# Wu-sm/Adversarial-Attacks-on-GAN-based-Image-Fusion

Hardware: AMD Instinct MI355X
Metric: attacked images/sec, PGD-20 L∞ ε=8/255 at 256², 1/2/4/8 MI355X (higher is better)
Workload: dtype f32; 1 GPU; PGD-20 L∞ eps=8/255 alpha=2/255 at 256², 128 images/GPU (BASELINE config #4 per-GPU share), RCCL all-gather of outputs when N>1; encoder=e4e, norm=linf, images_per_gpu=128, global_batch=128, size=256, pgd_steps=20, parallelism=dp1, dist_world_size=1, output_in_eps_ball_and_finite=True, fp32_arithmetic=fp32

## Files before the change

adversarial-attacks-on-gan-based-image-fusion_amd/csrc/conv_halo_x6.hip:

```cpp
#include "conv_common.h"
#include "halo_epilogue.h"

namespace mia {

#ifdef MIA_STAMPS
__device__ unsigned long long g_x6_stamps[4][16];
#endif

template <int BN_, int TPS_ = 1>
struct HaloX6 {
  static constexpr int PH = 16, PW = 16, NW = 8, NT = 64 * NW;
  static constexpr int WN = BN_ == 128 ? 2 : 1, WM = NW / WN, FM = 16 / WM, FN = 4;
  static constexpr int BM = PH * PW, BN = BN_, BK = 32;
  static constexpr int HSIDE = PW + 2, HROWS = (PH + 2) * HSIDE;
  static constexpr int HPIECES = (HROWS + 7) / 8;
  static constexpr int HBUF = HPIECES * 1024;
  static constexpr int LROWB = 64, LBUF = HROWS * LROWB;
  static constexpr int TPS = TPS_, NG = (9 + TPS - 1) / TPS;
  static constexpr int BHM = BN * ROWB, BL = BN * LROWB, BSTAGE1 = BHM + BL;
  static constexpr int BSTAGE = TPS * BSTAGE1;
  static constexpr int BWAVES = 4, HWAVES = 4;
  static constexpr int B_HM_INS = BN / 8 / BWAVES;
  static constexpr int B_L_INS = BN / 16 / BWAVES;
  static constexpr int H_INS = (HPIECES + HWAVES - 1) / HWAVES;
  static constexpr int HSTEPS = (4 + TPS - 1) / TPS;
  static constexpr int H_PER_STEP = (H_INS + HSTEPS - 1) / HSTEPS;
  static constexpr int EROWS = 128, ES = BN + 4;
  static constexpr int LDS = 2 * HBUF + LBUF + 2 * BSTAGE;
  static_assert(WM * FM * 16 == BM && WN * FN * 16 == BN, "");
  static_assert(B_HM_INS * 8 * BWAVES == BN && B_L_INS * 16 * BWAVES == BN, "");
  static_assert(LDS <= 160 * 1024, "");
};

template <int BN_, bool PRO, int EPI, bool EARLY, bool PRIO, bool UNR, int TPS = 1>
__global__ __launch_bounds__(HaloX6<BN_>::NT, 2) void conv_halo_x6_kernel(const ConvK k) {
  static_assert(!UNR || (EARLY && PRIO && EPI != -2), "UNR: the EARLY + PRIO schedule, D[ch][px]");
  static_assert(UNR || TPS == 1, "several taps per K-step: the unrolled loop only");
  typedef HaloX6<BN_, TPS> TL;
  constexpr int NG = TL::NG;
  constexpr int FM = TL::FM, FN = TL::FN, WN = TL::WN, NT = TL::NT, BN = TL::BN, BK = TL::BK;
  constexpr int HSIDE = TL::HSIDE, HROWS = TL::HROWS, HPIECES = TL::HPIECES, HBUF = TL::HBUF;
  constexpr int H_INS = TL::H_INS, HPS = TL::H_PER_STEP, HWAVES = TL::HWAVES;
  constexpr int B_HM_INS = TL::B_HM_INS, B_L_INS = TL::B_L_INS, BSTAGE = TL::BSTAGE;

  extern __shared__ __attribute__((aligned(16))) char smem[];
  char* const hbuf = smem;
  char* const lbuf = smem + 2 * HBUF;
  char* const bring = lbuf + TL::LBUF;

  const mia_conv_args& p = k.a;
  const int tid = threadIdx.x, lane = tid & 63;
  const int wid = __builtin_amdgcn_readfirstlane(tid >> 6);
  const int wm = wid / WN, wn = wid % WN;
  const ConvGroup G = k.g[0];
  const int H = p.H, W = p.W, Cin = p.Cin, Cout = p.Cout, Kpad = G.kpad;
  const int bl = xcd_remap(blockIdx.x, k.nblk);
  const int mt = bl / k.nbn, n0 = (bl % k.nbn) * BN;
  const int ptx = W / TL::PW, pty = H / TL::PH;
  const int x0 = (mt % ptx) * TL::PW;
  const int y0 = ((mt / ptx) % pty) * TL::PH;
  const int n = mt / (ptx * pty);

  const float* __restrict__ X = (const float*)p.x;
  const unsigned* __restrict__ Whm = (const unsigned*)G.w_split;
  const __bf16* __restrict__ Wl = (const __bf16*)(Whm + (size_t)Cout * Kpad);
  const char* zero = (const char*)g_zero16;
  const bool bwave = wid < TL::BWAVES;
  const int hw = wid - TL::BWAVES;
  const int my_pieces = bwave ? 0 : (HPIECES - hw + HWAVES - 1) / HWAVES;
#ifdef MIA_STAMPS
  const unsigned long long st_t0 = __builtin_amdgcn_s_memtime();
  const unsigned long long st_r0 = __builtin_amdgcn_s_memrealtime();
  unsigned long long st_pro = 0, st_cv = 0, st_wb = 0;
#endif

  constexpr int NSRC = H_INS > B_HM_INS + B_L_INS ? H_INS : B_HM_INS + B_L_INS;
  const char* src[NSRC];
#pragma unroll
  for (int j = 0; j < NSRC; ++j) {
    src[j] = nullptr;
    if (bwave) {
      if (j < B_HM_INS) {
        const int row = (wid * B_HM_INS + j) * 8 + (lane >> 3);
        const int c = EPI >= 0 ? min(n0 + row, Cout - 1) : n0 + row;
        if (c < Cout)
          src[j] = (const char*)(Whm + (size_t)c * Kpad + ((lane & 7) ^ fsw(row)) * 4);
      } else if (j < B_HM_INS + B_L_INS) {
        const int row = (wid * B_L_INS + j - B_HM_INS) * 16 + (lane >> 2);
        const int c = EPI >= 0 ? min(n0 + row, Cout - 1) : n0 + row;
        if (c < Cout)
          src[j] = (const char*)(Wl + (size_t)c * Kpad + ((lane & 3) ^ (lsw(row) >> 1)) * 8);
      }
    } else if (j < H_INS) {
      const int hr = (hw + HWAVES * j) * 8 + (lane >> 3);
      const int hy = hr / HSIDE, hx = hr - (hr / HSIDE) * HSIDE;
      const int y = y0 + hy - 1, x = x0 + hx - 1;
      if (hr < HROWS && y >= 0 && y < H && x >= 0 && x < W)
        src[j] = (const char*)(X + ((size_t)(n * H + y) * W + x) * Cin + ((lane & 7) ^ fsw(hr)) * 4);
    }
  }
  const int ncb = Cin / BK, nk = NG * ncb;

  auto issue_b = [&](int s, int st) {
    const int cb = s / NG, tg = s - (s / NG) * NG;
#pragma unroll
    for (int tt = 0; tt < TPS; ++tt) {
      const int t = tg * TPS + tt;
      if (TPS > 1 && t >= 9) break;
      const int koff = t * Cin + cb * BK;
      char* dst = bring + st * BSTAGE + tt * TL::BSTAGE1;
#pragma unroll
      for (int j = 0; j < B_HM_INS; ++j) {
        const char* a = EPI >= 0 ? src[j] + (size_t)koff * 4
                                 : src[j] ? src[j] + (size_t)koff * 4 : zero;
        __builtin_amdgcn_global_load_lds((gptr_t)a, (lptr_t)(dst + (wid * B_HM_INS + j) * 1024),
                                         16, 0, 0);
      }
#pragma unroll
      for (int j = 0; j < B_L_INS; ++j) {
        const char* a = EPI >= 0                ? src[B_HM_INS + j] + (size_t)koff * 2
                        : src[B_HM_INS + j] ? src[B_HM_INS + j] + (size_t)koff * 2
                                            : zero;
        __builtin_amdgcn_global_load_lds((gptr_t)a,
                                         (lptr_t)(dst + TL::BHM + (wid * B_L_INS + j) * 1024), 16,
                                         0, 0);
      }
    }
  };
  auto issue_h = [&](int cb, int j, int buf) {
    const char* a = src[j] ? src[j] + (size_t)cb * BK * 4 : zero;
    __builtin_amdgcn_global_load_lds((gptr_t)a,
                                     (lptr_t)(hbuf + buf * HBUF + (hw + HWAVES * j) * 1024), 16,
                                     0, 0);
  };
  const bool lrelu_in = p.act_in == MIA_ACT_LRELU_S2;
  auto convert = [&](int cb, int buf) {
    char* hb = hbuf + buf * HBUF;
    for (int c = tid; c < HROWS * 8; c += NT) {
      const int hr = c >> 3, pc = c & 7, lc = pc ^ fsw(hr);
      f32x4 v = *(const f32x4*)(hb + hr * ROWB + pc * 16);
      if constexpr (PRO) {
        const float mul = lrelu_in ? SQRT2 : 1.f;
        f32x4 s4 = {1.f, 1.f, 1.f, 1.f};
        if (p.in_scale) s4 = *(const f32x4*)(p.in_scale + (size_t)n * Cin + cb * BK + lc * 4);
#pragma unroll
        for (int e = 0; e < 4; ++e) {
          float f = v[e];
          if (lrelu_in) f = fmaxf(f, 0.2f * f);
          v[e] = f * (s4[e] * mul);
        }
      }
      u32x4 hm;
      u32x2 lo;
      split_quad(v, hm, lo);
      *(u32x4*)(hb + hr * ROWB + pc * 16) = hm;
      *(u32x2*)(lbuf + hr * TL::LROWB + ((lc ^ lsw(hr)) << 3)) = lo;
    }
  };

  if (bwave) {
    issue_b(0, 0);
  } else {
#pragma unroll
    for (int j = 0; j < H_INS; ++j)
      if (j < my_pieces) issue_h(0, j, 0);
  }
  asm volatile("s_waitcnt vmcnt(0)" ::: "memory");
  __syncthreads();
  convert(0, 0);
  __syncthreads();
#ifdef MIA_STAMPS
  st_pro = __builtin_amdgcn_s_memtime();
#endif

  f32x4 acc[FM][FN];
#pragma unroll
  for (int i = 0; i < FM; ++i)
#pragma unroll
    for (int j = 0; j < FN; ++j) acc[i][j] = f32x4{0.f, 0.f, 0.f, 0.f};

  const int frow = lane & 15, fq = lane >> 4;
  if constexpr (UNR) {
    int oh[FM + 2][3], ol[FM + 2][3];
#pragma unroll
    for (int q = 0; q < FM + 2; ++q)
#pragma unroll
      for (int c = 0; c < 3; ++c) {
        const int hr = (wm * FM + q) * HSIDE + frow + c;
        int vh = hr * ROWB + ((fq ^ fsw(hr)) << 4), vl = hr * TL::LROWB + ((fq ^ lsw(hr)) << 3);
        asm volatile("" : "+v"(vh), "+v"(vl));
        oh[q][c] = vh;
        ol[q][c] = vl;
      }
    int st = 0;
    for (int cb = 0; cb < ncb; ++cb) {
#pragma unroll
      for (int tg = 0; tg < NG; ++tg) {
        const int s = cb * NG + tg;
        int hoff = (cb & 1) * HBUF, x1 = 64, x2 = 32;
        asm volatile("" : "+s"(hoff), "+s"(x1), "+s"(x2));
        const char* ha = hbuf + hoff;
        const char* sb0 = bring + st * BSTAGE;
        if (bwave && s + 1 < nk) issue_b(s + 1, st ^ 1);
        if (!bwave && cb + 1 < ncb && tg < (H_INS + HPS - 1) / HPS) {
#pragma unroll
          for (int q = 0; q < HPS; ++q) {
            const int j = tg * HPS + q;
            if (j < H_INS && j < my_pieces) issue_h(cb + 1, j, (cb + 1) & 1);
          }
        }
#pragma unroll
        for (int tt = 0; tt < TPS; ++tt) {
          const int t = tg * TPS + tt;
          if (t >= 9) break;
          const int dy = t / 3, dx = t % 3;
          const char* sb = sb0 + tt * TL::BSTAGE1;
#pragma unroll
          for (int h = 0; h < 2; ++h) {
            const int ch = h * 4 + fq;
            u32x4 ahm[FM], bhm[FN];
            u32x2 al[FM], blo[FN];
#pragma unroll
            for (int i = 0; i < FM; ++i) {
              ahm[i] = *(const u32x4*)(ha + (h ? oh[i + dy][dx] ^ x1 : oh[i + dy][dx]));
              al[i] = *(const u32x2*)(lbuf + (h ? ol[i + dy][dx] ^ x2 : ol[i + dy][dx]));
            }
#pragma unroll
            for (int j = 0; j < FN; ++j) {
              const int row = wn * FN * 16 + 16 * j + frow;
              bhm[j] = *(const u32x4*)(sb + row * ROWB + ((ch ^ fsw(row)) << 4));
              blo[j] = *(const u32x2*)(sb + TL::BHM + row * TL::LROWB + ((ch ^ lsw(row)) << 3));
            }
            __builtin_amdgcn_s_setprio(1);
#pragma unroll
            for (int i = 0; i < FM; ++i)
#pragma unroll
              for (int j = 0; j < FN; ++j)
                acc[i][j] = mfma_x6(bhm[j], blo[j], ahm[i], al[i], acc[i][j]);
            __builtin_amdgcn_s_setprio(0);
          }
        }
#ifdef MIA_STAMPS
        const unsigned long long w0 = __builtin_amdgcn_s_memtime();
#endif
        if (bwave || tg == NG - 1) asm volatile("s_waitcnt vmcnt(0)" ::: "memory");
        __builtin_amdgcn_s_waitcnt(0xc07f);
        __builtin_amdgcn_s_barrier();
        __builtin_amdgcn_sched_barrier(0);
#ifdef MIA_STAMPS
        st_wb += __builtin_amdgcn_s_memtime() - w0;
#endif
        if (tg == NG - 1 && cb + 1 < ncb) {
#ifdef MIA_STAMPS
          const unsigned long long c0 = __builtin_amdgcn_s_memtime();
#endif
          convert(cb + 1, (cb + 1) & 1);
          __syncthreads();
#ifdef MIA_STAMPS
          st_cv += __builtin_amdgcn_s_memtime() - c0;
#endif
        }
        st ^= 1;
      }
    }
  } else {
  int st = 0, cb = 0, t = 0;
  for (int s = 0; s < nk; ++s) {
    const char* ha = hbuf + (cb & 1) * HBUF;
    const char* sb = bring + st * BSTAGE;
    const int dy = t >= 6 ? 2 : (t >= 3 ? 1 : 0), dx = t - 3 * dy;
    if (bwave && s + 1 < nk) issue_b(s + 1, st ^ 1);
    if constexpr (EARLY) {
      if (!bwave && cb + 1 < ncb) {
#pragma unroll
        for (int tt = 0; tt < (H_INS + HPS - 1) / HPS; ++tt) {
          if (t == tt) {
#pragma unroll
            for (int q = 0; q < HPS; ++q) {
              const int j = tt * HPS + q;
              if (j < H_INS && j < my_pieces) issue_h(cb + 1, j, (cb + 1) & 1);
            }
          }
        }
      }
    }
#pragma unroll
    for (int h = 0; h < 2; ++h) {
      const int ch = h * 4 + fq;
      u32x4 ahm[FM], bhm[FN];
      u32x2 al[FM], blo[FN];
#pragma unroll
      for (int i = 0; i < FM; ++i) {
        const int hr = (wm * FM + i + dy) * HSIDE + frow + dx;
        ahm[i] = *(const u32x4*)(ha + hr * ROWB + ((ch ^ fsw(hr)) << 4));
        al[i] = *(const u32x2*)(lbuf + hr * TL::LROWB + ((ch ^ lsw(hr)) << 3));
      }
#pragma unroll
      for (int j = 0; j < FN; ++j) {
        const int row = wn * FN * 16 + 16 * j + frow;
        bhm[j] = *(const u32x4*)(sb + row * ROWB + ((ch ^ fsw(row)) << 4));
        blo[j] = *(const u32x2*)(sb + TL::BHM + row * TL::LROWB + ((ch ^ lsw(row)) << 3));
      }
      if constexpr (PRIO) __builtin_amdgcn_s_setprio(1);
#pragma unroll
      for (int i = 0; i < FM; ++i)
#pragma unroll
        for (int j = 0; j < FN; ++j)
          acc[i][j] = EPI != -2 ? mfma_x6(bhm[j], blo[j], ahm[i], al[i], acc[i][j])
                                : mfma_x6(ahm[i], al[i], bhm[j], blo[j], acc[i][j]);
      if constexpr (PRIO) __builtin_amdgcn_s_setprio(0);
      if (!EARLY && h == 0 && !bwave && cb + 1 < ncb) {
        __builtin_amdgcn_sched_barrier(0);
#pragma unroll
        for (int tt = 0; tt < (H_INS + HPS - 1) / HPS; ++tt) {
          if (t == tt) {
#pragma unroll
            for (int q = 0; q < HPS; ++q) {
              const int j = tt * HPS + q;
              if (j < H_INS && j < my_pieces) issue_h(cb + 1, j, (cb + 1) & 1);
            }
          }
        }
        __builtin_amdgcn_sched_barrier(0);
      }
    }
#ifdef MIA_STAMPS
    const unsigned long long w0 = __builtin_amdgcn_s_memtime();
#endif
    if (bwave || t == 8) asm volatile("s_waitcnt vmcnt(0)" ::: "memory");
    __builtin_amdgcn_s_waitcnt(0xc07f);
    __builtin_amdgcn_s_barrier();
    __builtin_amdgcn_sched_barrier(0);
#ifdef MIA_STAMPS
    st_wb += __builtin_amdgcn_s_memtime() - w0;
#endif
    if (t == 8 && cb + 1 < ncb) {
#ifdef MIA_STAMPS
      const unsigned long long c0 = __builtin_amdgcn_s_memtime();
#endif
      convert(cb + 1, (cb + 1) & 1);
      __syncthreads();
#ifdef MIA_STAMPS
      st_cv += __builtin_amdgcn_s_memtime() - c0;
#endif
    }
    st ^= 1;
    if (++t == 9) { t = 0; ++cb; }
  }
  }
#ifdef MIA_STAMPS
  const unsigned long long st_loop = __builtin_amdgcn_s_memtime();
#endif
  if constexpr (EPI >= 0) {
    halo_epilogue_f<float, TL, EPI>(k, acc, n, y0, x0, n0, wm, wn, lane, -1, -1, nullptr,
                                    k.prered ? (float*)smem : nullptr, TL::WM, TL::BN);
  } else if constexpr (EPI == -1) {
    halo_epilogue<float, TL>(k, acc, n, y0, x0, n0, wm, wn, lane);
  } else {
    __syncthreads();
    const int img_row = n * H + y0;
    conv_epilogue<float, TL>(k, G, acc, smem, n0, true, n, [=](int r) {
      return (img_row + (r >> 4)) * W + x0 + (r & 15);
    }, (y0 / TL::PH) * (W / TL::PW) + x0 / TL::PW);
  }
#ifdef MIA_STAMPS
  if (wid == 0 && lane == 0) {
    const unsigned long long t1 = __builtin_amdgcn_s_memtime();
    const unsigned long long r1 = __builtin_amdgcn_s_memrealtime();
    unsigned long long* g = g_x6_stamps[(BN_ == 128 ? 1 : 0) + (PRO ? 2 : 0)];
    atomicAdd(g + 0, 1ull);
    atomicAdd(g + 1, t1 - st_t0);
    atomicAdd(g + 2, st_pro - st_t0);
    atomicAdd(g + 3, st_cv);
    atomicAdd(g + 4, t1 - st_loop);
    atomicAdd(g + 5, r1 - st_r0);
    atomicAdd(g + 6, (unsigned long long)nk);
    atomicAdd(g + 7, st_wb);
  }
  if (wid == 4 && lane == 0) atomicAdd(&g_x6_stamps[(BN_ == 128 ? 1 : 0) + (PRO ? 2 : 0)][8], st_wb);
#endif
}

template <int BN_, bool PRO, int EPI, bool EARLY, bool PRIO = false, bool UNR = false,
          int TPS = 1>
static int launch_x6_e(ConvK& k, hipStream_t st) {
  typedef HaloX6<BN_, TPS> TL;
  k.nbn = (k.a.Cout + TL::BN - 1) / TL::BN;
  k.nblk = k.a.N * (k.a.H / TL::PH) * (k.a.W / TL::PW) * k.nbn;
  size_t lds = TL::LDS;
  lds = std::max(lds, (size_t)TL::EROWS * TL::ES * 4);
  lds = std::max(lds, (size_t)TL::NW * TL::BN * 4);
  auto fn = conv_halo_x6_kernel<BN_, PRO, EPI, EARLY, PRIO, UNR, TPS>;
  if (const int rc = ensure_dyn_lds((const void*)fn, 160 * 1024); rc != MIA_OK) return rc;
  k.prered = EPI >= 0 && (EPI & epi::CSUM);
  const int H = k.a.H, W = k.a.W;
  const int nslots = EPI >= 0    ? halo_red_slots(H, W, TL::FM, TL::WM, k.prered)
                     : EPI == -1 ? halo_red_slots(H, W, TL::FM, TL::WM, false)
                                 : (H / TL::PH) * (W / TL::PW);
  RedQ r;
  int rc = conv_red_begin(k, r, nslots, st);
  if (rc != MIA_OK) return rc;
  hipLaunchKernelGGL(fn, dim3(k.nblk), dim3(TL::NT), lds, st, k);
  rc = check_launch("conv_halo_x6");
  return rc != MIA_OK ? rc : red_finish(r, st);
}

template <int BN_, bool PRO, int EPI>
static int launch_x6_(ConvK& k, hipStream_t st) {
  if constexpr (EPI >= 0) {
    const int u = tune(T_X6_UNR);
    if constexpr (BN_ == 64) {
      if (u == 2) return launch_x6_e<BN_, PRO, EPI, true, true, true, 2>(k, st);
    }
    if (u != 0) return launch_x6_e<BN_, PRO, EPI, true, true, true>(k, st);
  }
  return launch_x6_e<BN_, PRO, EPI, true, true>(k, st);
}

struct HaloX6S {
  static constexpr int PH = 8, PW = 16, NW = 4, NT = 64 * NW;
  static constexpr int WN = 1, WM = 4, FM = 2, FN = 4;
  static constexpr int BM = PH * PW, BN = 64, BK = 32;
  static constexpr int HSIDE = PW + 2, HROWS = (PH + 2) * HSIDE;
  static constexpr int HPIECES = (HROWS + 7) / 8;
  static constexpr int HBUF = HPIECES * 1024;
  static constexpr int LROWB = 64, LBUF = HROWS * LROWB;
  static constexpr int BHM = BN * ROWB, BL = BN * LROWB, BSTAGE = BHM + BL;
  static constexpr int B_HM_INS = BN / 8 / NW, B_L_INS = BN / 16 / NW;
  static constexpr int H_INS = (HPIECES + NW - 1) / NW;
  static constexpr int EROWS = 128, ES = BN + 4;
  static constexpr int LDS = HBUF + LBUF + 2 * BSTAGE;
  static_assert(WM * FM * 16 == BM && WN * FN * 16 == BN, "");
  static_assert(B_HM_INS * 8 * NW == BN && B_L_INS * 16 * NW == BN, "");
  static_assert(LDS <= 80 * 1024, "two blocks per CU");
};

template <bool PRO, int EPI>
__global__ __launch_bounds__(HaloX6S::NT, 2) void conv_halo_x6s_kernel(const ConvK k) {
  static_assert(EPI >= 0, "the specialised register epilogues only");
  typedef HaloX6S TL;
  constexpr int FM = TL::FM, FN = TL::FN, NT = TL::NT, BN = TL::BN, BK = TL::BK;
  constexpr int HSIDE = TL::HSIDE, HROWS = TL::HROWS, HPIECES = TL::HPIECES;
  constexpr int H_INS = TL::H_INS, B_HM_INS = TL::B_HM_INS, B_L_INS = TL::B_L_INS;
  constexpr int BSTAGE = TL::BSTAGE;

  extern __shared__ __attribute__((aligned(16))) char smem[];
  char* const hbuf = smem;
  char* const lbuf = smem + TL::HBUF;
  char* const bring = lbuf + TL::LBUF;

  const mia_conv_args& p = k.a;
  const int tid = threadIdx.x, lane = tid & 63;
  const int wid = __builtin_amdgcn_readfirstlane(tid >> 6);
  const int wm = wid, wn = 0;
  const ConvGroup G = k.g[0];
  const int H = p.H, W = p.W, Cin = p.Cin, Cout = p.Cout, Kpad = G.kpad;
  const int bl = xcd_remap(blockIdx.x, k.nblk);
  const int mt = bl / k.nbn, n0 = (bl % k.nbn) * BN;
  const int ptx = W / TL::PW, pty = H / TL::PH;
  const int x0 = (mt % ptx) * TL::PW;
  const int y0 = ((mt / ptx) % pty) * TL::PH;
  const int n = mt / (ptx * pty);

  const float* __restrict__ X = (const float*)p.x;
  const unsigned* __restrict__ Whm = (const unsigned*)G.w_split;
  const __bf16* __restrict__ Wl = (const __bf16*)(Whm + (size_t)Cout * Kpad);
  const char* zero = (const char*)g_zero16;

  const char* wsrc[B_HM_INS + B_L_INS];
#pragma unroll
  for (int j = 0; j < B_HM_INS + B_L_INS; ++j) {
    if (j < B_HM_INS) {
      const int row = (wid * B_HM_INS + j) * 8 + (lane >> 3);
      const int c = min(n0 + row, Cout - 1);
      wsrc[j] = (const char*)(Whm + (size_t)c * Kpad + ((lane & 7) ^ fsw(row)) * 4);
    } else {
      const int row = (wid * B_L_INS + j - B_HM_INS) * 16 + (lane >> 2);
      const int c = min(n0 + row, Cout - 1);
      wsrc[j] = (const char*)(Wl + (size_t)c * Kpad + ((lane & 3) ^ (lsw(row) >> 1)) * 8);
    }
  }
  const char* hsrc[H_INS];
#pragma unroll
  for (int j = 0; j < H_INS; ++j) {
    hsrc[j] = nullptr;
    const int hr = (wid + TL::NW * j) * 8 + (lane >> 3);
    const int hy = hr / HSIDE, hx = hr - (hr / HSIDE) * HSIDE;
    const int y = y0 + hy - 1, x = x0 + hx - 1;
    if (hr < HROWS && y >= 0 && y < H && x >= 0 && x < W)
      hsrc[j] = (const char*)(X + ((size_t)(n * H + y) * W + x) * Cin + ((lane & 7) ^ fsw(hr)) * 4);
  }
  const int ncb = Cin / BK, nk = 9 * ncb;

  auto issue_b = [&](int s, int st) {
    const int cb = s / 9, t = s - (s / 9) * 9;
// ... 138 lines not shown
  return rc != MIA_OK ? rc : red_finish(r, st);
}

constexpr int X6S_NONE = 1;
static int launch_x6s(ConvK& k, hipStream_t st, bool pro) {
  using namespace epi;
  const int f = epi_mask(k);
  if (pro) {
    if (f == (OSC | NOISE | BIAS | LRELU)) return launch_x6s_<true, OSC | NOISE | BIAS | LRELU>(k, st);
    return X6S_NONE;
  }
  switch (f) {
    case 0: return launch_x6s_<false, 0>(k, st);
    case BIAS: return launch_x6s_<false, BIAS>(k, st);
    case BIAS | RELU: return launch_x6s_<false, BIAS | RELU>(k, st);
    case PRELU: return launch_x6s_<false, PRELU>(k, st);
    case MASK: return launch_x6s_<false, MASK>(k, st);
    case TAP: return launch_x6s_<false, TAP>(k, st);
    case TAP | MASK: return launch_x6s_<false, TAP | MASK>(k, st);
    case ACC: return launch_x6s_<false, ACC>(k, st);
    case MASK | MSL: return launch_x6s_<false, MASK | MSL>(k, st);
    default: return X6S_NONE;
  }
}

template <int BN_, bool PRO>
static int launch_x6_spec(ConvK& k, hipStream_t st) {
  using namespace epi;
  const int f = epi_mask(k);
  if constexpr (PRO) {
    if (f == (OSC | NOISE | BIAS | LRELU))
      return launch_x6_<BN_, PRO, OSC | NOISE | BIAS | LRELU>(k, st);
  } else if constexpr (BN_ == 64) {
    switch (f) {
      case 0: return launch_x6_<BN_, PRO, 0>(k, st);
      case BIAS: return launch_x6_<BN_, PRO, BIAS>(k, st);
      case BIAS | RELU: return launch_x6_<BN_, PRO, BIAS | RELU>(k, st);
      case PRELU: return launch_x6_<BN_, PRO, PRELU>(k, st);
      case MASK: return launch_x6_<BN_, PRO, MASK>(k, st);
      case TAP: return launch_x6_<BN_, PRO, TAP>(k, st);
      case ACC: return launch_x6_<BN_, PRO, ACC>(k, st);
      case MASK | MSL: return launch_x6_<BN_, PRO, MASK | MSL>(k, st);
      default: break;
    }
  } else {
    switch (f) {
      case 0: return launch_x6_<BN_, PRO, 0>(k, st);
      case BIAS: return launch_x6_<BN_, PRO, BIAS>(k, st);
      case BIAS | RELU: return launch_x6_<BN_, PRO, BIAS | RELU>(k, st);
      case PRELU: return launch_x6_<BN_, PRO, PRELU>(k, st);
      case MASK: return launch_x6_<BN_, PRO, MASK>(k, st);
      case TAP: return launch_x6_<BN_, PRO, TAP>(k, st);
      case ACC: return launch_x6_<BN_, PRO, ACC>(k, st);
      case MASK | MSL: return launch_x6_<BN_, PRO, MASK | MSL>(k, st);
      case OSC | SDOT: return launch_x6_<BN_, PRO, OSC | SDOT>(k, st);
      case OSC | SDOT | BAB: return launch_x6_<BN_, PRO, OSC | SDOT | BAB>(k, st);
      default: break;
    }
  }
  return launch_x6_<BN_, PRO, -1>(k, st);
}

bool conv_halo_x6_eligible(const ConvK& k, int dtype) {
#ifdef MIA_F32_NATIVE
  (void)k;
  (void)dtype;
  return false;
#endif
  if (tune(T_CONV_X6) == 0) return false;
  const mia_conv_args& a = k.a;
  const ConvGroup& G = k.g[0];
  return dtype == MIA_F32 && G.w_split != nullptr && k.ng == 1 && k.stride == 1 && G.kh == 3 &&
         G.kw == 3 && G.pad_y == 1 && G.pad_x == 1 && G.ho == a.H && G.wo == a.W && G.ay == 1 &&
         G.ax == 1 && G.by == 0 && G.bx == 0 && !a.shuffle_out && a.H % 16 == 0 &&
         a.W % 16 == 0 && a.Cin % 32 == 0 && k.HT == a.H && k.WT == a.W &&
         a.Cout >= 64;
}

#ifdef MIA_STAMPS
extern "C" int mia_debug_x6_stamps(unsigned long long* host, int reset) {
  if (hipMemcpyFromSymbol(host, HIP_SYMBOL(g_x6_stamps), sizeof(g_x6_stamps)) != hipSuccess)
    return 1;
  if (reset) {
    static const unsigned long long zero[4][16] = {};
    if (hipMemcpyToSymbol(HIP_SYMBOL(g_x6_stamps), zero, sizeof(zero)) != hipSuccess) return 1;
  }
  return 0;
}
#endif

int launch_conv_halo_x6(ConvK& k, hipStream_t st) {
  const bool pro = k.a.in_scale != nullptr || k.a.act_in != MIA_ACT_NONE;
#ifdef MIA_STAMPS
  {
    static int seen[64];
    static int nseen = 0;
    const int key = (epi_mask(k) << 2) | (pro ? 2 : 0) | (k.a.Cout == 64 ? 1 : 0);
    bool found = false;
    for (int i = 0; i < nseen; ++i) found |= seen[i] == key;
    if (!found && nseen < 64) {
      seen[nseen++] = key;
      fprintf(stderr, "x6 launch: Cout %d pro %d epi_mask %d (%dx%d Cin %d)\n", k.a.Cout, pro,
              epi_mask(k), k.a.H, k.a.W, k.a.Cin);
    }
  }
#endif
  const int sel = tune(T_HALO_EPI);
  if (k.a.Cout == 64 && sel == 1 && tune(T_X6_64S) != 0 && k.a.H % HaloX6S::PH == 0) {
    const int rc = launch_x6s(k, st, pro);
    if (rc != X6S_NONE) return rc;
  }
  if (k.a.Cout == 64) {
    if (sel == 0) return pro ? launch_x6_<64, true, -2>(k, st) : launch_x6_<64, false, -2>(k, st);
    if (sel == 1) return pro ? launch_x6_spec<64, true>(k, st) : launch_x6_spec<64, false>(k, st);
    return pro ? launch_x6_<64, true, -1>(k, st) : launch_x6_<64, false, -1>(k, st);
  }
  if (sel == 0) return pro ? launch_x6_<128, true, -2>(k, st) : launch_x6_<128, false, -2>(k, st);
  if (sel == 1) return pro ? launch_x6_spec<128, true>(k, st) : launch_x6_spec<128, false>(k, st);
  return pro ? launch_x6_<128, true, -1>(k, st) : launch_x6_<128, false, -1>(k, st);
}

}
```

adversarial-attacks-on-gan-based-image-fusion_amd/csrc/conv_wres.hip:

```cpp
#include "conv_common.h"
#include "halo_epilogue.h"

namespace mia {

template <int NW_, int WN_>
struct WresTileT {
  static constexpr int NW = NW_, WN = WN_, WM = NW / WN, FM = 16 / WM, FN = 4 / WN, NT = 64 * NW;
  static constexpr int PH = 16, PW = 16, HSIDE = PW + 2, HROWS = (PH + 2) * HSIDE;
  static constexpr int HPIECES = (HROWS + 7) / 8;
  static constexpr int HBUF = HPIECES * 8 * ROWB;
  static constexpr int H_INS = (HPIECES + NW - 1) / NW;
  static constexpr int CPP = 2 * FN;
  static constexpr int AUXW = FM * 16 * CPP * 16;
  static_assert(WM * FM == PH && WN * FN == 4, "");
};
typedef WresTileT<8, 2> WresTile;

template <int EPI>
struct WresAux {
  static constexpr bool TAP = EPI & epi::TAP, MASK = (EPI & epi::MASK) && !TAP;
  static constexpr bool ACC = EPI & epi::ACC;
  static constexpr int N = TAP ? 2 : (MASK ? 1 : 0) + (ACC ? 1 : 0);
  static_assert(N <= 2 && (TAP || N <= 1), "prefetched operands per wave");
  static_assert(!(EPI & (epi::SDOT | epi::BAB | epi::NOISE)), "not a weights-resident epilogue");
// ... 404 lines not shown
    for (int t = 0; t < 9; ++t) {
      const int dy = t / 3, dx = t - 3 * (t / 3);
      VT af[FM];
#pragma unroll
      for (int i = 0; i < FM; ++i) {
        const int hr = (wid * FM + i + dy) * HSIDE + fr + dx;
        af[i] = *(const VT*)(ha + hr * TL::RB + ((fq ^ sw32(hr)) << 4));
      }
#pragma unroll
      for (int i = 0; i < FM; ++i)
#pragma unroll
        for (int j = 0; j < FN; ++j)
          acc[i][j] = mfma_chunk<T>(wreg[t][j], af[i], acc[i][j]);
    }
    if constexpr (NZ || BB) {
#pragma unroll
      for (int i = 0; i < FM; ++i) {
        if constexpr (NZ) R.nz[i] = p.noise_w * R.nz[i];
        if constexpr (BB) R.bnz[i] = p.bab_noise_w * R.bnz[i];
      }
    }
    EpiChan<FN> E;
    {
      const int cl = (lane >> 4) << 2;
#pragma unroll
      for (int j = 0; j < FN; ++j) {
        const f32x4* r = (const f32x4*)(ctab + cl + 16 * j);
        E.osc[j] = r[0];
        E.bia[j] = r[8];
        E.dmv[j] = r[16];
        E.bbv[j] = r[24];
        E.msl[j] = r[32];
        E.asl[j] = r[40];
      }
    }
    halo_epilogue_f<T, TL, EPI>(k, acc, n, y0, x0, 0, wid, 0, lane, -1, -1, PRE ? &R : nullptr,
                                red, NW, 32, nullptr, &E);
    if (more) {
      if constexpr (PRO) {
        const int n1 = (tile + 1) / (ptx * pty);
        if (n1 != sn) {
          set_style(n1);
          sn = n1;
        }
      }
      store_halo(buf ^ 1);
    }
    buf ^= 1;
  }
}

static bool wres32_mask_ok(int f, bool pro) {
  using namespace epi;
  if (pro) return f == (OSC | NOISE | BIAS | LRELU);
  switch (f) {
    case OSC | SDOT: case OSC | SDOT | ACC: case OSC | SDOT | BAB: case OSC | SDOT | ACC | BAB:
    case 0: case ACC:
      return true;
    default:
      return false;
  }
}

bool conv_wres32_eligible(const ConvK& k, int dtype) {
  if (tune(T_CONV_WRES32) == 0) return false;
  const mia_conv_args& a = k.a;
  const ConvGroup& G = k.g[0];
  if (dtype == MIA_F32 || k.ng != 1 || k.stride != 1 || G.kh != 3 || G.kw != 3 || G.pad_y != 1 ||
      G.pad_x != 1 || G.ho != a.H || G.wo != a.W || G.ay != 1 || G.ax != 1 || G.by != 0 ||
      G.bx != 0 || a.shuffle_out || a.H % 16 != 0 || a.W % 16 != 0 || k.HT != a.H ||
      k.WT != a.W || k.ystride != a.Cout || a.Cin != 32 || a.Cout != 32 || G.kpad < 9 * 32 ||
      !a.y)
    return false;
  const bool pro = a.in_scale != nullptr;
  if (!pro && a.act_in != MIA_ACT_NONE) return false;
  if (pro && k.cout_mod != a.Cout) return false;
  return wres32_mask_ok(epi_mask(k), pro);
}

template <typename T, bool PRO, int EPI>
static int launch_wres32_(ConvK& k, hipStream_t st) {
  typedef Wres32Tile TL;
  auto fn = conv_wres32_kernel<T, PRO, EPI>;
  static const int occ = [&] {
    int o = 0;
    if (hipOccupancyMaxActiveBlocksPerMultiprocessor(&o, (const void*)fn, TL::NT, TL::LDS) !=
            hipSuccess || o < 1)
      o = 1;
    return o;
  }();
  const int per_cu = device_cu_count() * occ;
  const int ntiles = k.a.N * (k.a.H / TL::PH) * (k.a.W / TL::PW);
  const int grid = std::min(ntiles, per_cu);
  k.nbn = 1;
  k.nblk = ntiles;
  constexpr bool RED = (EPI & (epi::SDOT | epi::BAB | epi::CSUM)) != 0;
  k.prered = RED;
  RedQ r;
  int rc = conv_red_begin(k, r, halo_red_slots(k.a.H, k.a.W, TL::FM, TL::NW, k.prered), st);
  if (rc != MIA_OK) return rc;
  hipLaunchKernelGGL(fn, dim3(grid), dim3(TL::NT), TL::LDS, st, k);
  rc = check_launch("conv_wres32");
  return rc != MIA_OK ? rc : red_finish(r, st);
}

int launch_conv_wres32(ConvK& k, int dtype, hipStream_t st) {
  using namespace epi;
  const bool pro = k.a.in_scale != nullptr;
  MIA_DISPATCH_DTYPE(dtype, T, {
    if constexpr (sizeof(T) == 2) {
      if (pro) return launch_wres32_<T, true, OSC | NOISE | BIAS | LRELU>(k, st);
      switch (epi_mask(k)) {
        case OSC | SDOT: return launch_wres32_<T, false, OSC | SDOT>(k, st);
        case OSC | SDOT | ACC: return launch_wres32_<T, false, OSC | SDOT | ACC>(k, st);
        case OSC | SDOT | BAB: return launch_wres32_<T, false, OSC | SDOT | BAB>(k, st);
        case OSC | SDOT | ACC | BAB:
          return launch_wres32_<T, false, OSC | SDOT | ACC | BAB>(k, st);
        case 0: return launch_wres32_<T, false, 0>(k, st);
        case ACC: return launch_wres32_<T, false, ACC>(k, st);
        default: break;
      }
    }
  });
  return set_error("conv_wres32: no specialisation for this launch");
}

}
```

adversarial-attacks-on-gan-based-image-fusion_amd/csrc/mia_common.h:

```cpp
#pragma once
#include <hip/hip_runtime.h>
#include <stdint.h>
#include <string>

#include "../../include/miattack.h"

namespace mia {

typedef __attribute__((ext_vector_type(4))) float f32x4;
typedef __attribute__((ext_vector_type(8))) _Float16 f16x8;
typedef __attribute__((ext_vector_type(8))) __bf16 bf16x8;

template <typename T> struct Vec;
template <> struct Vec<float> { typedef f32x4 type; static constexpr int N = 4; };
template <> struct Vec<_Float16> { typedef f16x8 type; static constexpr int N = 8; };
template <> struct Vec<__bf16> { typedef bf16x8 type; static constexpr int N = 8; };

__device__ __forceinline__ float to_f(float v) { return v; }
__device__ __forceinline__ float to_f(_Float16 v) { return (float)v; }
__device__ __forceinline__ float to_f(__bf16 v) { return (float)v; }
template <typename T> __device__ __forceinline__ T from_f(float v);
template <> __device__ __forceinline__ float from_f<float>(float v) { return v; }
template <> __device__ __forceinline__ _Float16 from_f<_Float16>(float v) { return (_Float16)v; }
template <> __device__ __forceinline__ __bf16 from_f<__bf16>(float v) { return (__bf16)v; }

constexpr float SQRT2 = 1.41421356237309504880f;

__device__ __forceinline__ float lrelu_s2(float v) { return (v > 0.f ? v : 0.2f * v) * SQRT2; }
__device__ __forceinline__ float lrelu_s2_grad(float pre) { return pre > 0.f ? SQRT2 : 0.2f * SQRT2; }
__device__ __forceinline__ float lrelu_s2_inv_grad(float pre) {
  return pre > 0.f ? 0.70710678118654752f : 3.5355339059327376f;
}

#define MIA_DPP(v, ctrl) \
  __builtin_bit_cast(float, __builtin_amdgcn_mov_dpp(__builtin_bit_cast(int, (v)), (ctrl), 0xf, 0xf, false))
__device__ __forceinline__ void lds_handoff() {
  asm volatile("s_waitcnt lgkmcnt(0)\n\ts_barrier" ::: "memory");
}

__device__ __forceinline__ float row16_sum(float v) {
  v += MIA_DPP(v, 0xB1);
  v += MIA_DPP(v, 0x4E);
  v += MIA_DPP(v, 0x141);
  v += MIA_DPP(v, 0x140);
  return v;
}

__device__ __forceinline__ float wave_sum(float v) {
#pragma unroll
  for (int o = 32; o > 0; o >>= 1) v += __shfl_xor(v, o, 64);
  return v;
}

int set_error(const std::string& msg);
int check_launch(const char* what);

int device_cu_count();
int ensure_dyn_lds(const void* fn, int bytes);

enum TuneKey {
  T_CONV_HALO,
  T_CONV_X6,
  T_HALO_EPI,
  T_X6_UNR,
  T_CONV_THIN,
  T_CONV_THIN32,
  T_CONV_WRES,
  T_CONV_REGEPI,
  T_CONV_SMALLTILE,
  T_S2DG_X6,
  T_S2DG_HALO,
  T_UPCONV_X6,
  T_UPCONV_HALO,
  T_CONV_WRES32,
  T_HALO_C64,
  T_X6_64S,
  T_UPCONV_X6S,
  T_CONV_WRES128,
  T_NKEYS
};
int tune(TuneKey key);

struct RedQ {
  float* dst[3];
  float* part;
  int nslots, count;
};
float* red_scratch(hipStream_t st, size_t bytes);
int red_begin(RedQ& r, float* d0, float* d1, float* d2, int nslots, int count, hipStream_t st,
              bool zero = false);
int red_finish(const RedQ& r, hipStream_t st);

__device__ __forceinline__ void red_store(float* part, int nslots, int count, int q, int slot,
                                          int i, float v) {
  part[((size_t)q * nslots + slot) * count + i] = v;
}

}

#define MIA_DISPATCH_DTYPE(dtype, T, ...)                                   \
  switch (dtype) {                                                          \
    case MIA_F32: { typedef float T; __VA_ARGS__; break; }                  \
    case MIA_F16: { typedef _Float16 T; __VA_ARGS__; break; }               \
    case MIA_BF16: { typedef __bf16 T; __VA_ARGS__; break; }                \
    default: return mia::set_error("unsupported dtype");                    \
  }

#define MIA_CHECK_ARG(cond, msg) \
  do { if (!(cond)) return mia::set_error(std::string(__func__) + ": " + (msg)); } while (0)
```

adversarial-attacks-on-gan-based-image-fusion_amd/csrc/reduce.hip:

```cpp
#include <algorithm>
#include <cstdlib>
#include <cstring>
#include <mutex>
#include <unordered_map>
#include <vector>

#include "mia_common.h"

namespace mia {

namespace {
struct Scratch {
  float* p = nullptr;
  size_t bytes = 0;
};
std::mutex g_mu;
std::unordered_map<hipStream_t, Scratch> g_scratch;
}

namespace {
struct TuneDef {
  const char* name;
  int value;
};
TuneDef g_tune[T_NKEYS] = {
    {"MIA_CONV_HALO", 1}, {"MIA_CONV_X6", 1},       {"MIA_HALO_EPI", 1},    {"MIA_X6_UNR", 2},
    {"MIA_CONV_THIN", 1}, {"MIA_CONV_THIN32", 1},   {"MIA_CONV_WRES", 1},
    {"MIA_CONV_REGEPI", 1},   {"MIA_CONV_SMALLTILE", 512},
    {"MIA_S2DG_X6", 1},   {"MIA_S2DG_HALO", 1},     {"MIA_UPCONV_X6", 1},   {"MIA_UPCONV_HALO", 1},
    {"MIA_CONV_WRES32", 1},
    {"MIA_HALO_C64", 1},  {"MIA_X6_64S", 1},
    {"MIA_UPCONV_X6S", 1}, {"MIA_CONV_WRES128", 1}};
std::once_flag g_tune_once;
void tune_init() {
  for (auto& d : g_tune) {
    const char* e = getenv(d.name);
    if (e && *e) d.value = atoi(e);
  }
}
}

int tune(TuneKey key) {
  std::call_once(g_tune_once, tune_init);
  return g_tune[key].value;
}

namespace {
std::mutex g_dev_mu;
std::unordered_map<int, int> g_ncu;
std::unordered_map<const void*, std::vector<int>> g_lds_set;
int current_device() {
  int dev = 0;
  (void)hipGetDevice(&dev);
  return dev;
}
}

int device_cu_count() {
  const int dev = current_device();
  std::lock_guard<std::mutex> lock(g_dev_mu);
  auto it = g_ncu.find(dev);
  if (it != g_ncu.end()) return it->second;
  int ncu = 0;
  if (hipDeviceGetAttribute(&ncu, hipDeviceAttributeMultiprocessorCount, dev) != hipSuccess ||
      ncu <= 0)
    ncu = 256;
  g_ncu[dev] = ncu;
  return ncu;
}

int ensure_dyn_lds(const void* fn, int bytes) {
  const int dev = current_device();
  std::lock_guard<std::mutex> lock(g_dev_mu);
  std::vector<int>& done = g_lds_set[fn];
  if (std::find(done.begin(), done.end(), dev) != done.end()) return MIA_OK;
  if (hipFuncSetAttribute(fn, hipFuncAttributeMaxDynamicSharedMemorySize, bytes) != hipSuccess)
    return set_error("hipFuncSetAttribute(MaxDynamicSharedMemorySize) failed");
  done.push_back(dev);
  return MIA_OK;
}

float* red_scratch(hipStream_t st, size_t bytes) {
  std::lock_guard<std::mutex> lock(g_mu);
  Scratch& s = g_scratch[st];
  if (s.bytes >= bytes) return s.p;
  if (s.p) {
    if (hipStreamSynchronize(st) != hipSuccess || hipFree(s.p) != hipSuccess) return nullptr;
    s.p = nullptr;
    s.bytes = 0;
  }
  size_t want = bytes < (1u << 20) ? (1u << 20) : bytes;
  want = want + want / 4;
  void* p = nullptr;
  if (hipMalloc(&p, want) != hipSuccess) return nullptr;
  s.p = (float*)p;
  s.bytes = want;
  return s.p;
}

constexpr int RED_CHUNK = 64;
static inline int red_nchunks(int nslots) { return nslots <= 2 * RED_CHUNK ? 1 : (nslots + RED_CHUNK - 1) / RED_CHUNK; }

int red_begin(RedQ& r, float* d0, float* d1, float* d2, int nslots, int count, hipStream_t st,
              bool zero) {
  r.dst[0] = d0;
  r.dst[1] = d1;
  r.dst[2] = d2;
  r.nslots = nslots;
  r.count = count;
  r.part = nullptr;
  if (!d0 && !d1 && !d2) return MIA_OK;
  if (nslots < 1 || count < 1) return set_error("red_begin: empty reduction");
  const int nch = red_nchunks(nslots);
  const size_t part_bytes = (size_t)3 * nslots * count * sizeof(float);
  const size_t bytes = part_bytes + (nch > 1 ? (size_t)3 * nch * count * sizeof(float) : 0);
  r.part = red_scratch(st, bytes);
  if (!r.part) return set_error("red_begin: scratch allocation failed");
  if (zero && hipMemsetAsync(r.part, 0, part_bytes, st) != hipSuccess)
    return set_error("red_begin: memset failed");
  return MIA_OK;
}

__device__ __forceinline__ float ordered_sum(const float* __restrict__ src, int n, int stride) {
  float s = 0.f;
  int k = 0;
  for (; k + 8 <= n; k += 8) {
    float t[8];
#pragma unroll
    for (int u = 0; u < 8; ++u) t[u] = src[(size_t)(k + u) * stride];
#pragma unroll
    for (int u = 0; u < 8; ++u) s += t[u];
  }
  for (; k < n; ++k) s += src[(size_t)k * stride];
  return s;
}

__global__ __launch_bounds__(256) void red_finish_kernel(const float* __restrict__ part,
                                                         float* d0, float* d1, float* d2,
                                                         int nslots, int count) {
  const int q = blockIdx.y;
  float* dst = q == 0 ? d0 : (q == 1 ? d1 : d2);
  if (!dst) return;
  const int i = blockIdx.x * 256 + threadIdx.x;
  if (i >= count) return;
  const float* src = part + (size_t)q * nslots * count + i;
  dst[i] += ordered_sum(src, nslots, count);
}

__global__ __launch_bounds__(256) void red_chunk_kernel(const float* __restrict__ part,
                                                        float* __restrict__ tmp, int has0,
                                                        int has1, int has2, int nslots,
                                                        int count) {
  const int q = blockIdx.z, c = blockIdx.y;
  if (!(q == 0 ? has0 : (q == 1 ? has1 : has2))) return;
  const int i = blockIdx.x * 256 + threadIdx.x;
  if (i >= count) return;
  const int k0 = c * RED_CHUNK, k1 = min(k0 + RED_CHUNK, nslots);
  const float* src = part + ((size_t)q * nslots + k0) * count + i;
  tmp[((size_t)q * gridDim.y + c) * count + i] = ordered_sum(src, k1 - k0, count);
}

int red_finish(const RedQ& r, hipStream_t st) {
// ... 84 lines not shown
```

Before: 17.56 attacked images/s.

## Add staggered x6 conv loop where halo waves lag weight waves by half a step

Adds a staggered variant of the unrolled 128-column x6 halo conv main loop. The weight-loading waves read operands before their MFMAs, as before. The halo waves run their MFMAs first and then read the next half-step's operands, so the two wave groups hit LDS reads and MFMA at different times instead of contending in lockstep. It is enabled by default for non-prologue launches through a new tuning key whose default ignores the environment. The change also caches the wres32 occupancy query per device, where before it was a single function-local static, and adds more timing stamps. The cost is added register pressure and schedule complexity, with a risk of ordering hazards around the shared-memory handoff.

```diff
diff --git a/adversarial-attacks-on-gan-based-image-fusion_amd/csrc/conv_halo_x6.hip b/adversarial-attacks-on-gan-based-image-fusion_amd/csrc/conv_halo_x6.hip
--- a/adversarial-attacks-on-gan-based-image-fusion_amd/csrc/conv_halo_x6.hip
+++ b/adversarial-attacks-on-gan-based-image-fusion_amd/csrc/conv_halo_x6.hip
@@ -1,10 +1,12 @@
+#include <type_traits>
+
 #include "conv_common.h"
 #include "halo_epilogue.h"
 
 namespace mia {
 
 #ifdef MIA_STAMPS
-__device__ unsigned long long g_x6_stamps[4][16];
+__device__ unsigned long long g_x6_stamps[4][24];
 #endif
 
 template <int BN_, int TPS_ = 1>
@@ -32,10 +34,11 @@
   static_assert(LDS <= 160 * 1024, "");
 };
 
-template <int BN_, bool PRO, int EPI, bool EARLY, bool PRIO, bool UNR, int TPS = 1>
+template <int BN_, bool PRO, int EPI, bool EARLY, bool PRIO, bool UNR, int TPS = 1, int STG = 0>
 __global__ __launch_bounds__(HaloX6<BN_>::NT, 2) void conv_halo_x6_kernel(const ConvK k) {
   static_assert(!UNR || (EARLY && PRIO && EPI != -2), "UNR: the EARLY + PRIO schedule, D[ch][px]");
   static_assert(UNR || TPS == 1, "several taps per K-step: the unrolled loop only");
+  static_assert(STG == 0 || (UNR && TPS == 1 && BN_ == 128), "staggered loop: the 128-column tile");
   typedef HaloX6<BN_, TPS> TL;
   constexpr int NG = TL::NG;
   constexpr int FM = TL::FM, FN = TL::FN, WN = TL::WN, NT = TL::NT, BN = TL::BN, BK = TL::BK;
@@ -72,6 +75,7 @@
   const unsigned long long st_t0 = __builtin_amdgcn_s_memtime();
   const unsigned long long st_r0 = __builtin_amdgcn_s_memrealtime();
   unsigned long long st_pro = 0, st_cv = 0, st_wb = 0;
+  unsigned long long st_rd = 0, st_m0 = 0, st_arr = 0, st_rel = 0;
 #endif
 
   constexpr int NSRC = H_INS > B_HM_INS + B_L_INS ? H_INS : B_HM_INS + B_L_INS;
@@ -193,6 +197,113 @@
         ol[q][c] = vl;
       }
     int st = 0;
+    if constexpr (STG != 0) {
+      auto loop = [&](auto lagc) {
+      constexpr bool lag = decltype(lagc)::value;
+      u32x4 ahm[FM], bhm[FN];
+      u32x2 al[FM], blo[FN];
+      auto mfmas = [&] {
+        __builtin_amdgcn_s_setprio(1);
+#pragma unroll
+        for (int i = 0; i < FM; ++i)
+#pragma unroll
+          for (int j = 0; j < FN; ++j)
+            acc[i][j] = mfma_x6(bhm[j], blo[j], ahm[i], al[i], acc[i][j]);
+        __builtin_amdgcn_s_setprio(0);
+      };
+      for (int cb = 0; cb < ncb; ++cb) {
+#pragma unroll
+        for (int tg = 0; tg < NG; ++tg) {
+          const int s = cb * NG + tg;
+          int hoff = (cb & 1) * HBUF, x1 = 64, x2 = 32;
+          asm volatile("" : "+s"(hoff), "+s"(x1), "+s"(x2));
+          const char* ha = hbuf + hoff;
+          const char* sb = bring + st * BSTAGE;
+          const int dy = tg / 3, dx = tg % 3;
+#ifdef MIA_STAMPS
+          const unsigned long long t_top = __builtin_amdgcn_s_memtime();
+          unsigned long long t_rd = 0, t_m0 = 0;
+#endif
+          if (!lag && s + 1 < nk) issue_b(s + 1, st ^ 1);
+#pragma unroll
+          for (int h = 0; h < 2; ++h) {
+            auto reads = [&] {
+              const int ch = h * 4 + fq;
+#pragma unroll
+              for (int i = 0; i < FM; ++i) {
+                ahm[i] = *(const u32x4*)(ha + (h ? oh[i + dy][dx] ^ x1 : oh[i + dy][dx]));
+                al[i] = *(const u32x2*)(lbuf + (h ? ol[i + dy][dx] ^ x2 : ol[i + dy][dx]));
+              }
+#pragma unroll
+              for (int j = 0; j < FN; ++j) {
+                const int row = wn * FN * 16 + 16 * j + frow;
+                bhm[j] = *(const u32x4*)(sb + row * ROWB + ((ch ^ fsw(row)) << 4));
+                blo[j] = *(const u32x2*)(sb + TL::BHM + row * TL::LROWB + ((ch ^ lsw(row)) << 3));
+              }
+            };
+            if constexpr (!lag) {
+#ifdef MIA_STAMPS
+              if (h == 0) t_rd = __builtin_amdgcn_s_memtime();
+#endif
+              reads();
+            }
+#ifdef MIA_STAMPS
+            if (h == 0) t_m0 = __builtin_amdgcn_s_memtime();
+#endif
+            if (tg == 0 && h == 0) {
+              if (!(lag && cb == 0)) mfmas();
+            } else {
+              mfmas();
+            }
+            if constexpr (lag) {
+              if (h == 0 && cb + 1 < ncb && tg < (H_INS + HPS - 1) / HPS) {
+#pragma unroll
+                for (int q = 0; q < HPS; ++q) {
+                  const int j = tg * HPS + q;
+                  if (j < H_INS && j < my_pieces) issue_h(cb + 1, j, (cb + 1) & 1);
+                }
+              }
+#ifdef MIA_STAMPS
+              if (h == 0) t_rd = __builtin_amdgcn_s_memtime();
+#endif
+              reads();
+            }
+          }
+#ifdef MIA_STAMPS
+          const unsigned long long w0 = __builtin_amdgcn_s_memtime();
+#endif
+          if (!lag || tg == NG - 1) asm volatile("s_waitcnt vmcnt(0)" ::: "memory");
+          lds_handoff();
+          __builtin_amdgcn_sched_barrier(0);
+#ifdef MIA_STAMPS
+          {
+            const unsigned long long t_end = __builtin_amdgcn_s_memtime();
+            st_wb += t_end - w0;
+            st_rd += t_rd - t_top;
+            st_m0 += t_m0 - t_top;
+            st_arr += w0 - t_top;
+            st_rel += t_end - t_top;
+          }
+#endif
+          if (tg == NG - 1 && cb + 1 < ncb) {
+#ifdef MIA_STAMPS
+            const unsigned long long c0 = __builtin_amdgcn_s_memtime();
+#endif
+            convert(cb + 1, (cb + 1) & 1);
+            __syncthreads();
+#ifdef MIA_STAMPS
+            st_cv += __builtin_amdgcn_s_memtime() - c0;
+#endif
+          }
+          st ^= 1;
+        }
+      }
+      if constexpr (lag) mfmas();
+      };
+      static_assert(TL::BWAVES == 4, "the weight waves lead, the halo waves lag");
+      if (bwave) loop(std::false_type{});
+      else loop(std::true_type{});
+    } else {
     for (int cb = 0; cb < ncb; ++cb) {
 #pragma unroll
       for (int tg = 0; tg < NG; ++tg) {
@@ -201,6 +312,10 @@
         asm volatile("" : "+s"(hoff), "+s"(x1), "+s"(x2));
         const char* ha = hbuf + hoff;
         const char* sb0 = bring + st * BSTAGE;
+#ifdef MIA_STAMPS
+        const unsigned long long t_top = __builtin_amdgcn_s_memtime();
+        unsigned long long t_rd = 0, t_m0 = 0;
+#endif
         if (bwave && s + 1 < nk) issue_b(s + 1, st ^ 1);
         if (!bwave && cb + 1 < ncb && tg < (H_INS + HPS - 1) / HPS) {
 #pragma unroll
@@ -220,6 +335,9 @@
             const int ch = h * 4 + fq;
             u32x4 ahm[FM], bhm[FN];
             u32x2 al[FM], blo[FN];
+#ifdef MIA_STAMPS
+            if (tt == 0 && h == 0) t_rd = __builtin_amdgcn_s_memtime();
+#endif
 #pragma unroll
             for (int i = 0; i < FM; ++i) {
               ahm[i] = *(const u32x4*)(ha + (h ? oh[i + dy][dx] ^ x1 : oh[i + dy][dx]));
@@ -232,6 +350,9 @@
               blo[j] = *(const u32x2*)(sb + TL::BHM + row * TL::LROWB + ((ch ^ lsw(row)) << 3));
             }
             __builtin_amdgcn_s_setprio(1);
+#ifdef MIA_STAMPS
+            if (tt == 0 && h == 0) t_m0 = __builtin_amdgcn_s_memtime();
+#endif
 #pragma unroll
             for (int i = 0; i < FM; ++i)
 #pragma unroll
@@ -248,7 +369,14 @@
         __builtin_amdgcn_s_barrier();
         __builtin_amdgcn_sched_barrier(0);
 #ifdef MIA_STAMPS
-        st_wb += __builtin_amdgcn_s_memtime() - w0;
+        {
+          const unsigned long long t_end = __builtin_amdgcn_s_memtime();
+          st_wb += t_end - w0;
+          st_rd += t_rd - t_top;
+          st_m0 += t_m0 - t_top;
+          st_arr += w0 - t_top;
+          st_rel += t_end - t_top;
+        }
 #endif
         if (tg == NG - 1 && cb + 1 < ncb) {
 #ifdef MIA_STAMPS
@@ -262,6 +390,7 @@
         }
         st ^= 1;
       }
+    }
     }
   } else {
   int st = 0, cb = 0, t = 0;
@@ -378,11 +507,18 @@
     atomicAdd(g + 7, st_wb);
   }
   if (wid == 4 && lane == 0) atomicAdd(&g_x6_stamps[(BN_ == 128 ? 1 : 0) + (PRO ? 2 : 0)][8], st_wb);
+  if ((wid == 0 || wid == 4) && lane == 0) {
+    unsigned long long* g = g_x6_stamps[(BN_ == 128 ? 1 : 0) + (PRO ? 2 : 0)] + (wid ? 13 : 9);
+    atomicAdd(g + 0, st_rd);
+    atomicAdd(g + 1, st_m0);
+    atomicAdd(g + 2, st_arr);
+    atomicAdd(g + 3, st_rel);
+  }
 #endif
 }
 
 template <int BN_, bool PRO, int EPI, bool EARLY, bool PRIO = false, bool UNR = false,
-          int TPS = 1>
+          int TPS = 1, int STG = 0>
 static int launch_x6_e(ConvK& k, hipStream_t st) {
   typedef HaloX6<BN_, TPS> TL;
   k.nbn = (k.a.Cout + TL::BN - 1) / TL::BN;
@@ -390,7 +526,7 @@
   size_t lds = TL::LDS;
   lds = std::max(lds, (size_t)TL::EROWS * TL::ES * 4);
   lds = std::max(lds, (size_t)TL::NW * TL::BN * 4);
-  auto fn = conv_halo_x6_kernel<BN_, PRO, EPI, EARLY, PRIO, UNR, TPS>;
+  auto fn = conv_halo_x6_kernel<BN_, PRO, EPI, EARLY, PRIO, UNR, TPS, STG>;
   if (const int rc = ensure_dyn_lds((const void*)fn, 160 * 1024); rc != MIA_OK) return rc;
   k.prered = EPI >= 0 && (EPI & epi::CSUM);
   const int H = k.a.H, W = k.a.W;
@@ -405,12 +541,26 @@
   return rc != MIA_OK ? rc : red_finish(r, st);
 }
 
+constexpr bool x6_stagger_wins(bool pro, int epi) {
+#ifdef MIA_X6_STAGGER_ALL
+  return MIA_X6_STAGGER_ALL != 0;
+#else
+  (void)epi;
+  return !pro;
+#endif
+}
+
 template <int BN_, bool PRO, int EPI>
 static int launch_x6_(ConvK& k, hipStream_t st) {
   if constexpr (EPI >= 0) {
     const int u = tune(T_X6_UNR);
     if constexpr (BN_ == 64) {
       if (u == 2) return launch_x6_e<BN_, PRO, EPI, true, true, true, 2>(k, st);
+    }
+    if constexpr (BN_ == 128) {
+      const int sg = tune(T_X6_STAGGER);
+      if (u != 0 && (sg < 0 ? x6_stagger_wins(PRO, EPI) : sg != 0))
+        return launch_x6_e<BN_, PRO, EPI, true, true, true, 1, 1>(k, st);
     }
     if (u != 0) return launch_x6_e<BN_, PRO, EPI, true, true, true>(k, st);
   }
@@ -715,7 +865,7 @@
   if (hipMemcpyFromSymbol(host, HIP_SYMBOL(g_x6_stamps), sizeof(g_x6_stamps)) != hipSuccess)
     return 1;
   if (reset) {
-    static const unsigned long long zero[4][16] = {};
+    static const unsigned long long zero[4][24] = {};
     if (hipMemcpyToSymbol(HIP_SYMBOL(g_x6_stamps), zero, sizeof(zero)) != hipSuccess) return 1;
   }
   return 0;
diff --git a/adversarial-attacks-on-gan-based-image-fusion_amd/csrc/conv_wres.hip b/adversarial-attacks-on-gan-based-image-fusion_amd/csrc/conv_wres.hip
--- a/adversarial-attacks-on-gan-based-image-fusion_amd/csrc/conv_wres.hip
+++ b/adversarial-attacks-on-gan-based-image-fusion_amd/csrc/conv_wres.hip
@@ -510,14 +510,7 @@
 static int launch_wres32_(ConvK& k, hipStream_t st) {
   typedef Wres32Tile TL;
   auto fn = conv_wres32_kernel<T, PRO, EPI>;
-  static const int occ = [&] {
-    int o = 0;
-    if (hipOccupancyMaxActiveBlocksPerMultiprocessor(&o, (const void*)fn, TL::NT, TL::LDS) !=
-            hipSuccess || o < 1)
-      o = 1;
-    return o;
-  }();
-  const int per_cu = device_cu_count() * occ;
+  const int per_cu = device_cu_count() * max_blocks_per_cu((const void*)fn, TL::NT, TL::LDS);
   const int ntiles = k.a.N * (k.a.H / TL::PH) * (k.a.W / TL::PW);
   const int grid = std::min(ntiles, per_cu);
   k.nbn = 1;
diff --git a/adversarial-attacks-on-gan-based-image-fusion_amd/csrc/mia_common.h b/adversarial-attacks-on-gan-based-image-fusion_amd/csrc/mia_common.h
--- a/adversarial-attacks-on-gan-based-image-fusion_amd/csrc/mia_common.h
+++ b/adversarial-attacks-on-gan-based-image-fusion_amd/csrc/mia_common.h
@@ -57,6 +57,7 @@
 
 int device_cu_count();
 int ensure_dyn_lds(const void* fn, int bytes);
+int max_blocks_per_cu(const void* fn, int threads, size_t dyn_lds);
 
 enum TuneKey {
   T_CONV_HALO,
@@ -77,6 +78,7 @@
   T_X6_64S,
   T_UPCONV_X6S,
   T_CONV_WRES128,
+  T_X6_STAGGER,
   T_NKEYS
 };
 int tune(TuneKey key);
diff --git a/adversarial-attacks-on-gan-based-image-fusion_amd/csrc/reduce.hip b/adversarial-attacks-on-gan-based-image-fusion_amd/csrc/reduce.hip
--- a/adversarial-attacks-on-gan-based-image-fusion_amd/csrc/reduce.hip
+++ b/adversarial-attacks-on-gan-based-image-fusion_amd/csrc/reduce.hip
@@ -30,10 +30,11 @@
     {"MIA_S2DG_X6", 1},   {"MIA_S2DG_HALO", 1},     {"MIA_UPCONV_X6", 1},   {"MIA_UPCONV_HALO", 1},
     {"MIA_CONV_WRES32", 1},
     {"MIA_HALO_C64", 1},  {"MIA_X6_64S", 1},
-    {"MIA_UPCONV_X6S", 1}, {"MIA_CONV_WRES128", 1}};
+    {"MIA_UPCONV_X6S", 1}, {"MIA_CONV_WRES128", 1}, {"MIA_X6_STAGGER", -1}};
 std::once_flag g_tune_once;
 void tune_init() {
   for (auto& d : g_tune) {
+    if (&d == &g_tune[T_X6_STAGGER]) continue;
     const char* e = getenv(d.name);
     if (e && *e) d.value = atoi(e);
   }
@@ -78,6 +79,21 @@
     return set_error("hipFuncSetAttribute(MaxDynamicSharedMemorySize) failed");
   done.push_back(dev);
   return MIA_OK;
+}
+
+int max_blocks_per_cu(const void* fn, int threads, size_t dyn_lds) {
+  static std::unordered_map<const void*, std::unordered_map<int, int>> cache;
+  const int dev = current_device();
+  std::lock_guard<std::mutex> lock(g_dev_mu);
+  auto& per_dev = cache[fn];
+  auto it = per_dev.find(dev);
+  if (it != per_dev.end()) return it->second;
+  int occ = 0;
+  if (hipOccupancyMaxActiveBlocksPerMultiprocessor(&occ, fn, threads, dyn_lds) != hipSuccess ||
+      occ < 1)
+    occ = 1;
+  per_dev[dev] = occ;
+  return occ;
 }
 
 float* red_scratch(hipStream_t st, size_t bytes) {
```

New measurement: 17.89 attacked images/s (median of 6 runs). 1.9% higher.
